# wolearyc/ramannoodle

Measured on AMD Instinct MI355X. Metric: structures/sec (GNN polarizability eval), higher is better.
Workload: dtype f32

## Files before the change

### ramannoodle_amd/csrc/kernels_edge_ps.hip

```cpp
#include <algorithm>
#include <vector>

#include "fused_common.hpp"

namespace rn {

struct EdgePsArgs {
  const float *edge_in;
  float *edge_out;
  const float *node;
  const float *np3;
  float *agg_out;
  int *fail;
  int S;
  Graph g;
  Dims d;
  PassW<float> w;
};

#ifndef RN_PS_TIMING
#define RN_PS_TIMING 0
#endif
#ifndef RN_PS_PROBE
#define RN_PS_PROBE 0
#endif
#ifndef RN_PS_SLEEP
#define RN_PS_SLEEP 1
#endif
#ifndef RN_PS_PRIO
#define RN_PS_PRIO 3
#endif
#ifndef RN_PS_CPRIO
#define RN_PS_CPRIO 2
#endif
#ifndef RN_PS_LG8
#define RN_PS_LG8 1
#endif
#ifndef RN_PS_TICKET
#define RN_PS_TICKET 1
#endif
#ifndef RN_PS_LPRIO
#define RN_PS_LPRIO 1
#endif
#if RN_PS_TIMING
#define PS_T0() long long _t = (long long)__builtin_readcyclecounter(); ++tn
#define PS_TICK(i)                                                                       \
  do {                                                                                   \
    const long long _n = (long long)__builtin_readcyclecounter();                        \
    tl[(i) & 15] += (unsigned)(_n - _t);                                                 \
    _t = (long long)__builtin_readcyclecounter();                                        \
  } while (0)
#define PS_TFLUSH(first, last, shift)                                                    \
  do {                                                                                   \
    if (timed)                                                                           \
      for (int _i = (first); _i <= (last); ++_i) {                                       \
        tacc[2 * (_i + (shift))] += (long long)tl[_i & 15];                              \
        tacc[2 * (_i + (shift)) + 1] += (long long)tn;                                   \
      }                                                                                  \
  } while (0)
#else
#define PS_T0() do {} while (0)
#define PS_TICK(i) do {} while (0)
#define PS_TFLUSH(first, last, shift) do {} while (0)
#endif

namespace {
constexpr int PS_THREADS = 768;
constexpr int PS_PROD = 4;
constexpr int PS_ND = 16;
#ifndef RN_PS_NRT
#define RN_PS_NRT 8
#endif
constexpr int PS_NRT = RN_PS_NRT;
constexpr int PS_NRT_GRAM = 7;
constexpr int PS_GW = 3;
constexpr int PS_GSTRIDE = PS_GW * 16 * 16;
constexpr int PS_MAXNEW = 2;
constexpr int PS_TILE = 16 * FP;
constexpr int PS_BUF = (2 + PS_MAXNEW) * PS_TILE;

constexpr int PS_CSET = 4;
constexpr unsigned PS_FAILBIT = 0x80000000u;

enum { C_SPLIT = 0, C_NORM = 16, C_READY = 32, C_FREE0 = 48, C_FREE1 = 64, C_RD0 = 80, C_RD1 = 96, C_TICKET = 112 };

struct PsLds {
  size_t ring, qnp, bufP, bufC, atile, lnp, ints, sync, gram, total;
};
__host__ __device__ inline PsLds ps_lds(int maxR, int maxD, bool gram) {
  auto up = [](size_t b) { return (b + 15) & ~size_t(15); };
  const size_t maxR16 = ((size_t)maxR + 15) & ~size_t(15), rounds = ((size_t)maxD + PS_ND - 1) / PS_ND;
  PsLds L;
  size_t off = 0;
  const size_t ring_rows = (size_t)(gram ? PS_NRT_GRAM : PS_NRT) * 16;
  L.ring = off; off += ring_rows * LDQ * 4;
  L.qnp = off; off += ring_rows * 4 * 4;
  L.bufP = off; off += (size_t)2 * PS_ND * LDQ * 4;
  L.bufC = off; off += (size_t)2 * PS_ND * LDQ * 4;
  L.atile = off; off += ((size_t)2 * PS_BUF + PS_TILE) * 4;
  L.lnp = off; off += (size_t)(gram ? 6 : 16) * FP * 4;
  L.ints = off; off += up((maxR16 + 7 * (size_t)maxD + 2 * rounds + 8) * 4);
  L.sync = off; off += 128;
  L.gram = off; off += gram ? (size_t)2 * PS_PROD * PS_GSTRIDE * 4 : 0;
  L.total = off;
  return L;
}

struct PsStep {
  int has_dest;
  int u, r, g;
  int ntiles, tile0;
  int tu0, tt0, tu1, tt1;
  int slot0, slot1;
  int ubs;
};
struct PsSched {
  int nrounds, nrt, nunits;
  int P, pu, pt;
  int u, r, g;
  int h0, hc;
  int ring, ps, ubs;
};
__host__ __device__ inline int ps_wrap(int x, int ring) { return x >= ring ? x - ring : x; }
__host__ __device__ inline void ps_sched_init(PsSched &s, int nrounds, int nrt, int nunits, int hi0, int ring) {
  s.nrounds = nrounds;
  s.nrt = nrt;
  s.nunits = nunits;
  s.P = s.pu = s.pt = s.u = s.r = s.g = 0;
  s.h0 = s.hc = hi0;
  s.ring = ring;
  s.ps = s.ubs = 0;
}
__host__ __device__ inline void ps_sched_take(PsSched &s, PsStep &st, int n) {
  st.ntiles = n;
  st.tile0 = s.P;
  st.tu0 = st.tu1 = s.pu;
  st.tt0 = st.tt1 = s.pt;
  st.slot0 = st.slot1 = s.ps;
  if (n >= 1) {
    ++s.P;
    s.ps = ps_wrap(s.ps + 1, s.ring);
    if (++s.pt == s.nrt) { s.pt = 0; ++s.pu; }
  }
  if (n >= 2) {
    st.tu1 = s.pu;
    st.tt1 = s.pt;
    st.slot1 = s.ps;
    ++s.P;
    s.ps = ps_wrap(s.ps + 1, s.ring);
    if (++s.pt == s.nrt) { s.pt = 0; ++s.pu; }
  }
}
template <typename HiFn>
__host__ __device__ inline bool ps_sched_next(PsSched &s, HiFn hi, PsStep &st) {
  if (s.u >= s.nunits) return false;
  if (s.g == 0 && s.P < s.h0 + 1) {
    const int miss = s.h0 + 1 - s.P;
    st.has_dest = 0;
    st.u = st.r = st.g = 0;
    st.ubs = 0;
    ps_sched_take(s, st, miss < PS_MAXNEW ? miss : PS_MAXNEW);
    return true;
  }
  const int need_now = s.u * s.nrt + s.hc + 1;
  int u2 = s.u, r2 = s.r + 1;
  if (r2 == s.nrounds) { r2 = 0; ++u2; }
  const int h2 = r2 == 0 ? s.h0 : hi(r2);
  const int need_next = u2 < s.nunits ? u2 * s.nrt + h2 + 1 : need_now;
  int n = need_next - s.P;
  n = n < 0 ? 0 : (n > PS_MAXNEW ? PS_MAXNEW : n);
  if (n < need_now - s.P) n = need_now - s.P;
  st.has_dest = 1;
  st.u = s.u;
  st.r = s.r;
  st.g = s.g;
  st.ubs = s.ubs;
  ps_sched_take(s, st, n);
  if (u2 != s.u) {
    int b = s.ubs + s.nrt % s.ring;
    s.ubs = ps_wrap(b, s.ring);
  }
  s.u = u2;
  s.r = r2;
  s.hc = h2;
  ++s.g;
  return true;
}

__device__ __forceinline__ unsigned ps_wait_ge(unsigned word, unsigned target, unsigned ready_word, int *fail, int code) {
  for (unsigned spins = 0;; ++spins) {
    unsigned v;
    asm volatile("ds_read_b32 %0, %1\n\ts_waitcnt lgkmcnt(0)" : "=v"(v) : "v"(word) : "memory");
    v = (unsigned)__builtin_amdgcn_readfirstlane((int)v);
    if (v >= target) return v;
    bool give_up = spins > (1u << 21);
    if ((spins & 1023u) == 1023u && !give_up) {
      unsigned rv;
      asm volatile("ds_read_b32 %0, %1\n\ts_waitcnt lgkmcnt(0)" : "=v"(rv) : "v"(ready_word) : "memory");
      give_up = ((unsigned)__builtin_amdgcn_readfirstlane((int)rv) & PS_FAILBIT) != 0;
    }
    if (give_up) {
      *fail = code;
      asm volatile("ds_or_b32 %0, %1\n\ts_waitcnt vmcnt(0) lgkmcnt(0)" ::"v"(ready_word), "v"(PS_FAILBIT) : "memory");
      return v | PS_FAILBIT;
    }
#if RN_PS_SLEEP
    __builtin_amdgcn_s_sleep(RN_PS_SLEEP);
#endif
  }
}
__device__ __forceinline__ void ps_arrive(unsigned word, int lane) {
  asm volatile("s_waitcnt lgkmcnt(0)" ::: "memory");
  if (lane == 0) asm volatile("ds_add_u32 %0, %1" ::"v"(word), "v"(1u) : "memory");
}
__device__ __forceinline__ unsigned ps_arrive_ticket(unsigned word, int lane) {
  asm volatile("s_waitcnt lgkmcnt(0)" ::: "memory");
  unsigned old = 0;
  if (lane == 0) asm volatile("ds_add_rtn_u32 %0, %1, %2\n\ts_waitcnt lgkmcnt(0)" : "=&v"(old) : "v"(word), "v"(1u) : "memory");
  return (unsigned)__builtin_amdgcn_readfirstlane((int)old);
}
typedef __bf16 bf16x8 __attribute__((ext_vector_type(8)));
typedef __bf16 bf16x2 __attribute__((ext_vector_type(2)));
__device__ __forceinline__ void split_bf16x8(const f32x4 &x0, const f32x4 &x1, bf16x8 &hi, bf16x8 &lo) {
#pragma unroll
  for (int j = 0; j < 4; ++j) {
    const f32x2 v = j < 2 ? f32x2{x0[2 * j], x0[2 * j + 1]} : f32x2{x1[2 * j - 4], x1[2 * j - 3]};
    const bf16x2 h = __builtin_convertvector(v, bf16x2);
    const bf16x2 l = __builtin_convertvector(v - __builtin_convertvector(h, f32x2), bf16x2);
    hi[2 * j] = h[0];
    hi[2 * j + 1] = h[1];
    lo[2 * j] = l[0];
    lo[2 * j + 1] = l[1];
  }
}
__device__ __forceinline__ void ps_publish(unsigned word, unsigned value, int lane) {
  asm volatile("s_waitcnt lgkmcnt(0)" ::: "memory");
  if (lane == 0) asm volatile("ds_max_u32 %0, %1" ::"v"(word), "v"(value) : "memory");
}
}

template <bool PAD, bool PRE, bool GRAM, bool F16 = true>
__global__ __launch_bounds__(PS_THREADS) void edge_block_ps_kernel(EdgePsArgs a) {
  static_assert(F16 || (!PRE && !GRAM), "the exact-f32 instantiation keeps float32 rows and the in-loop cross term");
  extern __shared__ __attribute__((aligned(16))) unsigned char smem_raw[];
  constexpr int NRT = GRAM ? PS_NRT_GRAM : PS_NRT, RING = NRT * 16;
  constexpr bool LG8 = RN_PS_LG8 && !GRAM;
  constexpr unsigned CPR = LG8 ? 2u : (unsigned)PS_CSET;
  auto wrap_row = [](unsigned x) -> unsigned {
    if constexpr ((RING & (RING - 1)) == 0) return x & (unsigned)(RING - 1);
    else return min(x, x - (unsigned)RING);
  };
  const Graph &g = a.g;
  const PsLds L = ps_lds(g.pt_max_out_rows, g.pt_max_in_rows, GRAM);
  auto wsc = [&](int i) { return F16 ? a.w.mfma_scale_c[i] : 1.0f; };
  float *ring = reinterpret_cast<float *>(smem_raw + L.ring);
  float *qnp = reinterpret_cast<float *>(smem_raw + L.qnp);
  float *bufP = reinterpret_cast<float *>(smem_raw + L.bufP);
  float *bufC = reinterpret_cast<float *>(smem_raw + L.bufC);
  float *atile = reinterpret_cast<float *>(smem_raw + L.atile);
  float *na_tile = atile + 2 * PS_BUF;
  float *lnp = reinterpret_cast<float *>(smem_raw + L.lnp);
  float *s_c2b = lnp, *s_g3q = lnp + 2 * FP, *s_igp = lnp + 4 * FP;
  float *s_g3p = lnp + 6 * FP, *s_c21g = lnp + 8 * FP, *s_c21b = lnp + 10 * FP, *s_c22g = lnp + 12 * FP, *s_c22b = lnp + 13 * FP,
        *s_c3g = lnp + 14 * FP, *s_c3b = lnp + 15 * FP;
  int *ints = reinterpret_cast<int *>(smem_raw + L.ints);
  unsigned *sync = reinterpret_cast<unsigned *>(smem_raw + L.sync);
  const unsigned sync_a = lds_addr(sync);
  const unsigned atile_a = lds_addr(atile), lnp_a = lds_addr(lnp), qnp_a = lds_addr(qnp), ints_a = lds_addr(ints);
  const unsigned bufP_a = lds_addr(bufP), ring_a = lds_addr(ring);
  float *gram_f = reinterpret_cast<float *>(smem_raw + L.gram);
  const int maxD = g.pt_max_in_rows, maxR16 = (g.pt_max_out_rows + 15) & ~15;
  int *qb = ints;
  int *d_edge = qb + maxR16, *d_a = d_edge + maxD, *d_b = d_a + maxD, *d_rb = d_b + maxD, *d_cnt = d_rb + maxD,
      *d_skip = d_cnt + maxD, *d_re = d_skip + maxD;
  int *hi_t = d_re + maxD;
  int *lo_t = hi_t + (maxD + PS_ND - 1) / PS_ND;
  int *misc = lo_t + (maxD + PS_ND - 1) / PS_ND;
  const int hi_off = maxR16 + 7 * maxD;
  const int lo_off = hi_off + (maxD + PS_ND - 1) / PS_ND;

  const int tid = threadIdx.x, lane = tid & 63;
  const int wave = __builtin_amdgcn_readfirstlane(tid >> 6);
  const int l15 = lane & 15, quad = lane >> 4;

  int logical = blockIdx.x;
  if ((gridDim.x & 7) == 0) logical = (blockIdx.x & 7) * (gridDim.x >> 3) + (blockIdx.x >> 3);
  const int tile = logical % g.pt_num;
  const int sg = logical / g.pt_num, nsg = gridDim.x / g.pt_num;
  const int j0 = g.pt_begin[tile], j1 = g.pt_begin[tile + 1];
  const int eo0 = g.out_ptr[j0], R = g.out_ptr[j1] - eo0;
  const int di0 = g.in_ptr[j0], D = g.in_ptr[j1] - di0;
  const int nrounds = (D + PS_ND - 1) / PS_ND;
  const int back = g.pt_back;

  for (int c = tid; c < 2 * FP; c += PS_THREADS) {
    s_c2b[c] = a.w.c2_bias_c[c] * wsc(4);
    const float gam = a.w.c3_norm_1s.g[c];
    s_g3q[c] = gam * wsc(3);
    s_igp[c] = ((c % FP) < a.d.Fe) ? wsc(1) / gam * (1.0f / (float)a.d.Fe) : 0.0f;
    if constexpr (!GRAM) {
      s_g3p[c] = gam * wsc(1);
      s_c21g[c] = a.w.c2_norm_1.g[c];
      s_c21b[c] = a.w.c2_norm_1.b[c];
      if (c < FP) {
        s_c22g[c] = a.w.c2_norm_2.g[c];
        s_c22b[c] = a.w.c2_norm_2.b[c];
        s_c3g[c] = a.w.c3_norm_2.g[c];
        s_c3b[c] = a.w.c3_norm_2.b[c];
      }
    }
  }
  for (int r = tid; r < maxR16; r += PS_THREADS) qb[r] = g.edge_b[eo0 + min(r, max(R - 1, 0))];
  for (int i = tid; i < D; i += PS_THREADS) {
    const int dst = g.in_edge[di0 + i];
    const int ad = g.edge_a[dst], bd = g.edge_b[dst];
    const int rb = g.out_ptr[bd] - eo0, re = g.out_ptr[bd + 1] - eo0;
    const int rev = g.rev_edge[dst];
    d_edge[i] = dst;
    d_a[i] = ad;
    d_b[i] = bd;
    d_rb[i] = rb;
    d_cnt[i] = (re - rb) - (rev >= 0 ? 1 : 0);
    d_skip[i] = rev >= 0 ? rev - eo0 : re;
    d_re[i] = re;
  }
  if (tid < 32) sync[tid] = 0u;
  __syncthreads();
  if (tid < nrounds) {
    int top = 0, first = 1 << 30;
    const int last = min((tid + 1) * PS_ND, D);
    for (int i = 0; i < last; ++i) {
      top = max(top, d_re[i]);
      if (i >= tid * PS_ND && d_re[i] > d_rb[i]) first = min(first, d_rb[i]);
    }
    hi_t[tid] = (top + 15) / 16 - 1;
    lo_t[tid] = first == (1 << 30) ? (top + 15) / 16 : first / 16;
  }
  __syncthreads();
  if (tid == 0) misc[0] = max(hi_t[nrounds > 0 ? nrounds - 1 : 0] + 1, 1);
  __syncthreads();
  if (D == 0 || sg >= a.S) return;
  const int nrt = __builtin_amdgcn_readfirstlane(misc[0]);
  const int nunits = (a.S - sg + nsg - 1) / nsg;

  if (wave < PS_PROD) {
    __builtin_amdgcn_s_setprio(RN_PS_PRIO);
    const int colbase = wave * 32;
    auto uni = [](float v) { return __int_as_float(__builtin_amdgcn_readfirstlane(__float_as_int(v))); };
    const float s4 = uni(wsc(0));
    const float s5 = uni(wsc(2)), inv5 = uni(wsc(3));
    const float sc2 = uni(wsc(4));
    WaveB<F16> bW4, bW5, bWc;
    bW4.load(a.w.c3_WeT_c, 4 * FP, colbase, l15, quad, s4);
    bW5.load(a.w.c3_WeT_c + 2 * FP, 4 * FP, colbase, l15, quad, s5);
    bWc.load(a.w.c2_WT_c, 2 * FP, colbase, l15, quad, sc2);
    const float qscale = uni(inv5 * inv5 / (float)(2 * a.d.Fe));

    auto request = [&](const PsStep &st, int buf, int ln) {
      const int row = 4 * wave + (ln >> 4);
      const int piece = ((ln & 15) ^ row) & 15;
      float *dst = atile + buf * PS_BUF + wave * 256;
      const unsigned ia = ints_a + (unsigned)(maxR16 + min(st.r * PS_ND + row, D - 1)) * 4u;
      int de, da, db;
      lds_read1x3(ia, ia + (unsigned)maxD * 4u, ia + 2u * (unsigned)maxD * 4u, de, da, db);
      const int s = sg + st.u * nsg;
      const float *eb = a.edge_in + (int64_t)s * g.E * FP, *nb = a.node + (int64_t)s * g.N * FP;
      const float *eb0 = a.edge_in + (int64_t)(sg + min(st.tu0, nunits - 1) * nsg) * g.E * FP;
      const float *eb1 = a.edge_in + (int64_t)(sg + min(st.tu1, nunits - 1) * nsg) * g.E * FP;
      const unsigned r0 = (unsigned)(eo0 + min(st.tt0 * 16 + row, R - 1)), r1 = (unsigned)(eo0 + min(st.tt1 * 16 + row, R - 1));
      dma16(eb + ((unsigned)de * FP + 4 * piece), dst);
      dma16(nb + ((unsigned)db * FP + 4 * piece), dst + PS_TILE);
      dma16(nb + ((unsigned)da * FP + 4 * piece), na_tile + wave * 256);
      dma16(eb0 + (r0 * FP + 4 * piece), dst + 2 * PS_TILE);
      dma16(eb1 + (r1 * FP + 4 * piece), dst + 3 * PS_TILE);
    };
    auto split_landed = [&](int buf, int ln) {
      const int row = 4 * wave + (ln >> 4), phys = ln & 15;
      const unsigned tb = atile_a + (unsigned)(buf * PS_BUF) * 4u;
      const unsigned sa = tb + (unsigned)(wave * 256 + ln * 4) * 4u;
      f32x4 u, v, w;
      if constexpr (!PRE && F16) {
        lds_read3(sa, sa + 2 * PS_TILE * 4, sa + 3 * PS_TILE * 4, u, v, w);
        write_pair(tb, row, phys, u);
        write_pair(tb + 2 * PS_TILE * 4, row, phys, v);
        write_pair(tb + 3 * PS_TILE * 4, row, phys, w);
      }
      lds_read2(sa + PS_TILE * 4, atile_a + (unsigned)(2 * PS_BUF + wave * 256 + ln * 4) * 4u, u, v);
// ... 96 lines not shown
        asm volatile("global_load_dwordx4 %0, %1, off" : "=v"(qS[1]) : "v"(q_src + 16) : "memory");
      }
      if (cur.has_dest) {
        f32x4 accC[2];
        if constexpr (F16) {
          f16x8 ah[2], al[2];
          load_pair_a2(tb_a + PS_TILE * 4, l15, quad, ah, al, lnp_a + (unsigned)mycol * 4u, lnp_a + (unsigned)(mycol + 16) * 4u,
                       accC[0], accC[1]);
          if (!(RN_PS_PROBE & 2)) bWc.product_split(ah, al, accC);
        } else {
          float af[KS];
          load_f32_a2(tb_a + PS_TILE * 4, l15, quad, af, lnp_a + (unsigned)mycol * 4u, lnp_a + (unsigned)(mycol + 16) * 4u, accC[0], accC[1]);
          if (!(RN_PS_PROBE & 2)) bWc.product(af, accC);
        }
#pragma unroll
        for (int t = 0; t < 2; ++t)
          *reinterpret_cast<f32x4 *>(bufC + (slot0 + l15) * LDQ + mycol + 16 * t) = accC[t];
      }
      PS_TICK(6);
      const int ntl = (RN_PS_PROBE & 128) ? 0 : cur.ntiles;
      auto q_tile_finish = [&](f32x4 (&accQ)[2], const f32x4 (&g3v)[2], int ringrow) {
#pragma unroll
        for (int t = 0; t < 2; ++t) accQ[t] = qS[t] * s5 + accQ[t];
        float ss = 0.f;
#pragma unroll
        for (int t = 0; t < 2; ++t)
#pragma unroll
          for (int e = 0; e < 4; ++e) ss = fmaf(accQ[t][e], accQ[t][e], ss);
        ss = sum_xor32(sum_xor16(ss));
#pragma unroll
        for (int t = 0; t < 2; ++t) *reinterpret_cast<f32x4 *>(ring + ringrow * LDQ + mycol + 16 * t) = accQ[t] * g3v[t];
        if (quad == 0) qnp[ringrow * 4 + wave] = ss * qscale;
      };
      {
        f32x4 accQ[2] = {{0.f, 0.f, 0.f, 0.f}, {0.f, 0.f, 0.f, 0.f}}, g3v[2] = {{0.f, 0.f, 0.f, 0.f}, {0.f, 0.f, 0.f, 0.f}};
        if (ntl > 0) {
          if constexpr (F16) {
            f16x8 ah[2], al[2];
            load_pair_a2(tb_a + (unsigned)(2 * PS_TILE) * 4u, l15, quad, ah, al, lnp_a + (unsigned)(2 * FP + mycol) * 4u,
                         lnp_a + (unsigned)(2 * FP + mycol + 16) * 4u, g3v[0], g3v[1]);
            if (!(RN_PS_PROBE & 2)) bW5.product_split(ah, al, accQ);
          } else {
            float af[KS];
            load_f32_a2(tb_a + (unsigned)(2 * PS_TILE) * 4u, l15, quad, af, lnp_a + (unsigned)(2 * FP + mycol) * 4u,
                        lnp_a + (unsigned)(2 * FP + mycol + 16) * 4u, g3v[0], g3v[1]);
            if (!(RN_PS_PROBE & 2)) bW5.product(af, accQ);
          }
        }
        asm volatile("s_waitcnt vmcnt(0)" : "+v"(qS[0]), "+v"(qS[1]), "+v"(accQ[0]), "+v"(accQ[1])::"memory");
        PS_TICK(7);
        if (cur.has_dest && cur.g > back) {
          const int gdone = cur.g - back - 1;
          ps_wait_ge(sync_a + ((gdone & 1) ? C_RD1 : C_RD0), CPR * (unsigned)((gdone >> 1) + 1), sync_a + C_READY, a.fail, 3);
        }
        PS_TICK(9);
        if (ntl > 0) q_tile_finish(accQ, g3v, ringrow0);
      }
      if (ntl > 1) {
        const float *np3_q = a.np3 + (int64_t)(sg + min(cur.tu1, nunits - 1) * nsg) * g.N * (6 * FP);
        const unsigned oq = (unsigned)lds_read1(ints_a + (unsigned)min(cur.tt1 * 16 + l15, R - 1) * 4u) * (6 * FP) + mycol;
#pragma unroll
        for (int t = 0; t < 2; ++t) qS[t] = *reinterpret_cast<const f32x4 *>(np3_q + oq + 16 * t);
        f32x4 accQ[2] = {{0.f, 0.f, 0.f, 0.f}, {0.f, 0.f, 0.f, 0.f}}, g3v[2];
        if constexpr (F16) {
          f16x8 ah[2], al[2];
          load_pair_a2(tb_a + (unsigned)(3 * PS_TILE) * 4u, l15, quad, ah, al, lnp_a + (unsigned)(2 * FP + mycol) * 4u,
                       lnp_a + (unsigned)(2 * FP + mycol + 16) * 4u, g3v[0], g3v[1]);
          if (!(RN_PS_PROBE & 2)) bW5.product_split(ah, al, accQ);
        } else {
          float af[KS];
          load_f32_a2(tb_a + (unsigned)(3 * PS_TILE) * 4u, l15, quad, af, lnp_a + (unsigned)(2 * FP + mycol) * 4u,
                      lnp_a + (unsigned)(2 * FP + mycol + 16) * 4u, g3v[0], g3v[1]);
          if (!(RN_PS_PROBE & 2)) bW5.product(af, accQ);
        }
        q_tile_finish(accQ, g3v, cur.slot1 * 16 + l15);
      }
      if constexpr (GRAM) {
        if (cur.has_dest) {
          const unsigned prow_a = bufP_a + (unsigned)((slot0 + l15) * LDQ + mycol) * 4u;
          const unsigned ig_a = lnp_a + (unsigned)(4 * FP + mycol) * 4u;
          const int lo = __builtin_amdgcn_readfirstlane(lds_read1(ints_a + (unsigned)(lo_off + cur.r) * 4u));
          const int hiw = __builtin_amdgcn_readfirstlane(lds_read1(ints_a + (unsigned)(hi_off + cur.r) * 4u));
          unsigned qa[PS_GW];
#pragma unroll
          for (int k = 0; k < PS_GW; ++k) {
            int sl = cur.ubs + min(lo + k, max(hiw, lo));
            sl = sl >= NRT ? sl - NRT : sl;
            sl = sl >= NRT ? sl - NRT : sl;
            qa[k] = ring_a + (unsigned)((sl * 16 + l15) * LDQ + mycol) * 4u;
          }
          static_assert(PS_GW == 3, "the Gram phase is written for three window tiles");
          f32x4 p0, p1, i0, i1, q0[PS_GW], q1[PS_GW];
          asm volatile(
              "ds_read_b128 %0, %10\n\tds_read_b128 %1, %10 offset:64\n\tds_read_b128 %2, %11\n\tds_read_b128 %3, %11 offset:64\n\t"
              "ds_read_b128 %4, %12\n\tds_read_b128 %5, %12 offset:64\n\tds_read_b128 %6, %13\n\tds_read_b128 %7, %13 offset:64\n\t"
              "ds_read_b128 %8, %14\n\tds_read_b128 %9, %14 offset:64\n\ts_waitcnt lgkmcnt(0)"
              : "=&v"(p0), "=&v"(p1), "=&v"(i0), "=&v"(i1), "=&v"(q0[0]), "=&v"(q1[0]), "=&v"(q0[1]), "=&v"(q1[1]), "=&v"(q0[2]), "=&v"(q1[2])
              : "v"(prow_a), "v"(ig_a), "v"(qa[0]), "v"(qa[1]), "v"(qa[2])
              : "memory");
          bf16x8 ph, pl, qh[PS_GW], ql[PS_GW];
          split_bf16x8(p0 * i0, p1 * i1, ph, pl);
#pragma unroll
          for (int k = 0; k < PS_GW; ++k) split_bf16x8(q0[k], q1[k], qh[k], ql[k]);
          f32x4 gacc[PS_GW];
#pragma unroll
          for (int k = 0; k < PS_GW; ++k) gacc[k] = __builtin_amdgcn_mfma_f32_16x16x32_bf16(pl, qh[k], f32x4{0.f, 0.f, 0.f, 0.f}, 0, 0, 0);
#pragma unroll
          for (int k = 0; k < PS_GW; ++k) gacc[k] = __builtin_amdgcn_mfma_f32_16x16x32_bf16(ph, ql[k], gacc[k], 0, 0, 0);
#pragma unroll
          for (int k = 0; k < PS_GW; ++k) gacc[k] = __builtin_amdgcn_mfma_f32_16x16x32_bf16(ph, qh[k], gacc[k], 0, 0, 0);
          const int gout = ((cur.g & 1) * PS_PROD + wave) * PS_GSTRIDE + l15 * 16 + 4 * quad;
#pragma unroll
          for (int k = 0; k < PS_GW; ++k) *reinterpret_cast<f32x4 *>(gram_f + gout + k * 256) = gacc[k];
        }
      }
      PS_TICK(7);
      if (ps_arrive_ticket(sync_a + C_NORM, ln) == 4u * k + 3u) {
        if (ln < 16 * cur.ntiles) {
          const int rrow = ((ln >> 4) ? cur.slot1 : cur.slot0) * 16 + l15;
          f32x4 v, v2;
          lds_read2(qnp_a + (unsigned)rrow * 16u, qnp_a + (unsigned)rrow * 16u, v, v2);
          ring[rrow * LDQ + 2 * FP] = (v[0] + v[1]) + (v[2] + v[3]);
        }
        if (cur.has_dest) ps_publish(sync_a + C_READY, (unsigned)cur.g + 1u, ln);
      }
      PS_TICK(8);
      cur = nxt;
      have = have_next;
    }
    dma_wait();
    PS_TFLUSH(0, 9, 0);
    return;
  }

  const int cw = wave - PS_PROD;
  if constexpr (LG8) {
    const int l7 = lane & 7, grp = lane >> 3;
    const float inv2n = 1.0f / (float)(2 * a.d.Fe), invn = 1.0f / (float)a.d.Fe;
    const float spscale = wsc(1) * wsc(1) * inv2n;
    const float eps_c2 = 1e-5f * wsc(4) * wsc(4);
    int nval[2];
#pragma unroll
    for (int j = 0; j < 2; ++j) nval[j] = min(max(a.d.Fe - (4 * l7 + 32 * j), 0), 4);
    f32x2 bf2[2][2], bc2[2][2];
#pragma unroll
    for (int j = 0; j < 2; ++j) {
      const Vec4<float> bf = load4<float>(a.w.c3_norm_1s.b + 4 * l7 + 32 * j), bc = load4<float>(a.w.c3_norm_1s.b + FP + 4 * l7 + 32 * j);
      bf2[j][0] = f32x2{bf.v[0], bf.v[1]};
      bf2[j][1] = f32x2{bf.v[2], bf.v[3]};
      bc2[j][0] = f32x2{bc.v[0], bc.v[1]};
      bc2[j][1] = f32x2{bc.v[2], bc.v[3]};
      asm volatile("s_waitcnt vmcnt(0)" : "+v"(bf2[j][0]), "+v"(bf2[j][1]), "+v"(bc2[j][0]), "+v"(bc2[j][1]));
    }
    const float *ringc = ring + 4 * l7;
    const int sdelta = 2 * FP - 4 * l7;
    const unsigned total_rounds = (unsigned)nunits * (unsigned)nrounds;
    auto ln64 = [&](const Vec4<float> (&x)[2], const float *gt, const float *bt, Vec4<float> (&y)[2]) {
      float sum = 0.f;
#pragma unroll
      for (int j = 0; j < 2; ++j) sum += (x[j].v[0] + x[j].v[1]) + (x[j].v[2] + x[j].v[3]);
      const float mean = lg_sum<8>(sum) * invn;
      float dv[2][4], qq = 0.f;
#pragma unroll
      for (int j = 0; j < 2; ++j)
#pragma unroll
        for (int k = 0; k < 4; ++k) {
          dv[j][k] = x[j].v[k] - mean;
          if (PAD && k >= nval[j]) dv[j][k] = 0.f;
          qq = fmaf(dv[j][k], dv[j][k], qq);
        }
      const float rstd = fast_rsq(lg_sum<8>(qq) * invn + 1e-5f);
#pragma unroll
      for (int j = 0; j < 2; ++j) {
        const Vec4<float> gv = load4<float>(gt + 4 * l7 + 32 * j), bv = load4<float>(bt + 4 * l7 + 32 * j);
#pragma unroll
        for (int k = 0; k < 4; ++k) y[j].v[k] = dv[j][k] * rstd * gv.v[k] + bv.v[k];
      }
    };
    bool poisoned = false;
#if RN_PS_TIMING
    long long *tacc = reinterpret_cast<long long *>(a.fail + 16);
    const bool timed = blockIdx.x == 0 && (cw & 3) == 0 && lane == 0;
    unsigned tl[16] = {0, 0, 0, 0, 0, 0, 0, 0, 0, 0, 0, 0, 0, 0, 0, 0}, tn = 0;
#endif
    for (;;) {
      PS_T0();
      const unsigned tk = ps_arrive_ticket(sync_a + C_TICKET, lane);
      const unsigned gr = tk >> 1;
      if (gr >= total_rounds) break;
      const int slot = 8 * (int)(tk & 1u) + grp;
      const int u = (int)(gr / (unsigned)nrounds), r = (int)(gr - (unsigned)u * (unsigned)nrounds);
      const int ub = (int)(((unsigned)u * (unsigned)(nrt % NRT)) % (unsigned)NRT) * 16;
      poisoned |= (ps_wait_ge(sync_a + C_READY, gr + 1u, sync_a + C_READY, a.fail, 4) & PS_FAILBIT) != 0;
      PS_TICK(10);
      const int64_t erow0 = (int64_t)(sg + u * nsg) * g.E;
      const bool active = r * PS_ND + slot < D;
      const int i = min(r * PS_ND + slot, D - 1);
      const int64_t drow = erow0 + d_edge[i];
      f32x2 pf2[2][2], pc2[2][2], pdf2[2][2], pdc2[2][2];
      float spe;
      {
        const float *prow = bufP + ((int)(gr & 1u) * PS_ND + slot) * LDQ;
        float sp = 0.f;
#pragma unroll
        for (int j = 0; j < 2; ++j) {
          const int cj = 4 * l7 + 32 * j;
          const Vec4<float> xf = load4<float>(prow + cj), xc = load4<float>(prow + FP + cj);
          const Vec4<float> gf = load4<float>(s_g3p + cj), gc = load4<float>(s_g3p + FP + cj);
          const Vec4<float> jf = load4<float>(s_igp + cj), jc = load4<float>(s_igp + FP + cj);
#pragma unroll
          for (int k = 0; k < 4; ++k) sp += xf.v[k] * xf.v[k] + xc.v[k] * xc.v[k];
#pragma unroll
          for (int hh = 0; hh < 2; ++hh) {
            pdf2[j][hh] = f32x2{xf.v[2 * hh] * jf.v[2 * hh], xf.v[2 * hh + 1] * jf.v[2 * hh + 1]};
            pdc2[j][hh] = f32x2{xc.v[2 * hh] * jc.v[2 * hh], xc.v[2 * hh + 1] * jc.v[2 * hh + 1]};
            pf2[j][hh] = f32x2{xf.v[2 * hh] * gf.v[2 * hh], xf.v[2 * hh + 1] * gf.v[2 * hh + 1]};
            pc2[j][hh] = f32x2{xc.v[2 * hh] * gc.v[2 * hh], xc.v[2 * hh + 1] * gc.v[2 * hh + 1]};
          }
        }
        spe = lg_sum<8>(sp) * spscale + 1e-5f;
      }
      Vec4<float> c2v[2];
      {
        const float *crow = bufC + ((int)(gr & 1u) * PS_ND + slot) * LDQ;
        Vec4<float> xf[2], xc[2];
        float q = 0.f;
#pragma unroll
        for (int j = 0; j < 2; ++j) {
          xf[j] = load4<float>(crow + 4 * l7 + 32 * j);
          xc[j] = load4<float>(crow + FP + 4 * l7 + 32 * j);
#pragma unroll
          for (int k = 0; k < 4; ++k) q += xf[j].v[k] * xf[j].v[k] + xc[j].v[k] * xc[j].v[k];
        }
        const float rstd2 = fast_rsq(lg_sum<8>(q) * inv2n + eps_c2);
        Vec4<float> g2[2];
#pragma unroll
        for (int j = 0; j < 2; ++j) {
          const int cj = 4 * l7 + 32 * j;
          const Vec4<float> gf = load4<float>(s_c21g + cj), bf = load4<float>(s_c21b + cj);
          const Vec4<float> gc = load4<float>(s_c21g + FP + cj), bc = load4<float>(s_c21b + FP + cj);
#pragma unroll
          for (int k = 0; k < 4; ++k)
            g2[j].v[k] = (RN_PS_PROBE & 4) ? xf[j].v[k] + xc[j].v[k]
                                           : gate(xf[j].v[k] * rstd2 * gf.v[k] + bf.v[k], xc[j].v[k] * rstd2 * gc.v[k] + bc.v[k]);
        }
        if (RN_PS_PROBE & 4) {
          c2v[0] = g2[0];
          c2v[1] = g2[1];
        } else {
          ln64(g2, s_c22g, s_c22b, c2v);
        }
      }
      const int rb = d_rb[i], cnt = active ? d_cnt[i] : 0, rskip = d_skip[i];
      const int rbase = (int)wrap_row(wrap_row((unsigned)(ub + rb)));
      ps_arrive(sync_a + ((gr & 1u) ? C_FREE1 : C_FREE0), lane);
      PS_TICK(11);
      float acc[8] = {0.f, 0.f, 0.f, 0.f, 0.f, 0.f, 0.f, 0.f};
      {
        auto triplet = [&](const float *qr, float (&sumk)[8]) {
          f32x2 qf2[2][2], qc2[2][2];
#pragma unroll
          for (int j = 0; j < 2; ++j) {
            const float4 qfv = *reinterpret_cast<const float4 *>(qr + 32 * j), qcv = *reinterpret_cast<const float4 *>(qr + FP + 32 * j);
            qf2[j][0] = f32x2{qfv.x, qfv.y};
            qf2[j][1] = f32x2{qfv.z, qfv.w};
            qc2[j][0] = f32x2{qcv.x, qcv.y};
            qc2[j][1] = f32x2{qcv.z, qcv.w};
          }
          const float qs = qr[sdelta];
          f32x2 d2 = pdf2[0][0] * qf2[0][0], d3 = pdc2[0][0] * qc2[0][0];
          d2 = __builtin_elementwise_fma(pdf2[0][1], qf2[0][1], d2);
          d3 = __builtin_elementwise_fma(pdc2[0][1], qc2[0][1], d3);
          d2 = __builtin_elementwise_fma(pdf2[1][0], qf2[1][0], d2);
          d3 = __builtin_elementwise_fma(pdc2[1][0], qc2[1][0], d3);
          d2 = __builtin_elementwise_fma(pdf2[1][1], qf2[1][1], d2);
          d3 = __builtin_elementwise_fma(pdc2[1][1], qc2[1][1], d3);
          d2 += d3;
          const float dot = lg_sum<8>(d2.x + d2.y);
          float ve = dot + (spe + qs);
          ve = ve > 1e-5f ? ve : 1e-5f;
          const float rstd = fast_rsq(ve);
          const f32x2 rstd2 = {rstd, rstd}, one2 = {1.0f, 1.0f};
#pragma unroll
          for (int j = 0; j < 2; ++j)
#pragma unroll
            for (int hh = 0; hh < 2; ++hh) {
              const f32x2 xf2 = __builtin_elementwise_fma(pf2[j][hh] + qf2[j][hh], rstd2, bf2[j][hh]);
              const f32x2 xc2 = __builtin_elementwise_fma(pc2[j][hh] + qc2[j][hh], rstd2, bc2[j][hh]);
              const f32x2 e1 = {fast_exp2(xf2.x), fast_exp2(xf2.y)}, e2 = {fast_exp2(xc2.x), fast_exp2(xc2.y)};
              const f32x2 t2 = e2 + one2;
              const f32x2 den = __builtin_elementwise_fma(e1, t2, t2);
              const f32x2 rd = {fast_rcp(den.x), fast_rcp(den.y)};
              f32x2 sk = {sumk[4 * j + 2 * hh], sumk[4 * j + 2 * hh + 1]};
              sk = __builtin_elementwise_fma(e2 - one2, rd, sk);
              sumk[4 * j + 2 * hh] = sk.x;
              sumk[4 * j + 2 * hh + 1] = sk.y;
            }
        };
#if RN_PS_CPRIO
        __builtin_amdgcn_s_setprio(0);
#endif
        float acc2[8] = {0.f, 0.f, 0.f, 0.f, 0.f, 0.f, 0.f, 0.f};
        const int tskip = rskip - rb;
        auto row_of = [&](int t) { return ringc + __umul24(wrap_row((unsigned)(rbase + t + (t >= tskip ? 1 : 0))), (unsigned)LDQ); };
        int t = (RN_PS_PROBE & 1) ? cnt : 0;
        const int tmid = RN_PS_LPRIO ? ((cnt >> 1) & ~1) : 0;
        for (; t + 1 < tmid; t += 2) {
          triplet(row_of(t), acc);
          triplet(row_of(t + 1), acc2);
        }
#if RN_PS_LPRIO
        __builtin_amdgcn_s_setprio(RN_PS_LPRIO);
#endif
        for (; t + 1 < cnt; t += 2) {
          triplet(row_of(t), acc);
          triplet(row_of(t + 1), acc2);
        }
        if (t < cnt) triplet(row_of(t), acc);
#pragma unroll
        for (int k = 0; k < 8; ++k) acc[k] += acc2[k];
      }
      PS_TICK(12);
#if RN_PS_CPRIO
      __builtin_amdgcn_s_setprio(RN_PS_CPRIO);
#endif
      f32x4 old4[2];
#pragma unroll
      for (int j = 0; j < 2; ++j) {
        const int cj = 4 * l7 + 32 * j;
        if constexpr (PRE) {
          const char *pp = reinterpret_cast<const char *>(a.edge_in + drow * FP + (cj >> 3) * 8) + (cj & 7) * 2;
          const f16x4 hh = *reinterpret_cast<const f16x4 *>(pp), ll = *reinterpret_cast<const f16x4 *>(pp + 16);
#pragma unroll
          for (int k = 0; k < 4; ++k) old4[j][k] = (float)hh[k] + (float)ll[k];
        } else {
          old4[j] = *reinterpret_cast<const f32x4 *>(a.edge_in + drow * FP + cj);
        }
      }
      poisoned |= (ps_wait_ge(sync_a + ((gr & 1u) ? C_RD1 : C_RD0), CPR * (gr >> 1), sync_a + C_READY, a.fail, 6) & PS_FAILBIT) != 0;
      ps_arrive(sync_a + ((gr & 1u) ? C_RD1 : C_RD0), lane);
      if (active) {
        Vec4<float> a4[2], c3[2];
#pragma unroll
        for (int j = 0; j < 2; ++j) {
          a4[j] = Vec4<float>{{acc[4 * j], acc[4 * j + 1], acc[4 * j + 2], acc[4 * j + 3]}};
          if (a.agg_out) store4(a.agg_out + drow * FP + 4 * l7 + 32 * j, a4[j]);
        }
        if (RN_PS_PROBE & 4) {
          c3[0] = a4[0];
          c3[1] = a4[1];
        } else {
          ln64(a4, s_c3g, s_c3b, c3);
        }
#pragma unroll
        for (int j = 0; j < 2; ++j) {
          const int cj = 4 * l7 + 32 * j;
          f32x4 y;
#pragma unroll
          for (int k = 0; k < 4; ++k) {
            y[k] = (RN_PS_PROBE & 4) ? old4[j][k] + c2v[j].v[k] + c3[j].v[k] : fast_tanh(old4[j][k] + c2v[j].v[k] + c3[j].v[k]);
            if (poisoned) y[k] = __int_as_float(0x7fc00000);
          }
          if constexpr (PRE) {
            char *pp = reinterpret_cast<char *>(a.edge_out + drow * FP + (cj >> 3) * 8) + (cj & 7) * 2;
            f16x4 hh, ll;
#pragma unroll
            for (int k = 0; k < 4; ++k) {
              hh[k] = (_Float16)y[k];
              ll[k] = (_Float16)(y[k] - (float)hh[k]);
            }
            *reinterpret_cast<f16x4 *>(pp) = hh;
            *reinterpret_cast<f16x4 *>(pp + 16) = ll;
          } else {
            *reinterpret_cast<f32x4 *>(a.edge_out + drow * FP + cj) = y;
          }
        }
      }
      PS_TICK(13);
    }
    PS_TFLUSH(10, 13, (cw >> 2) ? 6 : 0);
    return;
  }
  const int cset = cw >> 2;
  const int c0 = 4 * l15;
  const int nvalid = min(max(a.d.Fe - c0, 0), 4);
  const float inv2n = 1.0f / (float)(2 * a.d.Fe), invn = 1.0f / (float)a.d.Fe;
  const float spscale = wsc(1) * wsc(1) * inv2n;
  const float eps_c2 = 1e-5f * wsc(4) * wsc(4);
  f32x2 bf2[2], bc2[2];
  {
    const Vec4<float> bf = load4<float>(a.w.c3_norm_1s.b + c0), bc = load4<float>(a.w.c3_norm_1s.b + FP + c0);
    bf2[0] = f32x2{bf.v[0], bf.v[1]};
    bf2[1] = f32x2{bf.v[2], bf.v[3]};
    bc2[0] = f32x2{bc.v[0], bc.v[1]};
    bc2[1] = f32x2{bc.v[2], bc.v[3]};
    asm volatile("s_waitcnt vmcnt(0)" : "+v"(bf2[0]), "+v"(bf2[1]), "+v"(bc2[0]), "+v"(bc2[1]));
  }
  LnParams<float> k_c3 = {load4<float>(a.w.c3_norm_2.g + c0), load4<float>(a.w.c3_norm_2.b + c0)};
  LnParams<float> k_c21f = {load4<float>(a.w.c2_norm_1.g + c0), load4<float>(a.w.c2_norm_1.b + c0)};
  LnParams<float> k_c21c = {load4<float>(a.w.c2_norm_1.g + FP + c0), load4<float>(a.w.c2_norm_1.b + FP + c0)};
  LnParams<float> k_c22 = {load4<float>(a.w.c2_norm_2.g + c0), load4<float>(a.w.c2_norm_2.b + c0)};
  Vec4<float> g3f = load4<float>(a.w.c3_norm_1s.g + c0), g3c = load4<float>(a.w.c3_norm_1s.g + FP + c0);
  {
    auto pin = [](Vec4<float> &x) { asm volatile("s_waitcnt vmcnt(0)" : "+v"(x.v[0]), "+v"(x.v[1]), "+v"(x.v[2]), "+v"(x.v[3])); };
    pin(k_c3.g); pin(k_c3.b); pin(k_c21f.g); pin(k_c21f.b); pin(k_c21c.g); pin(k_c21c.b); pin(k_c22.g); pin(k_c22.b);
    pin(g3f); pin(g3c);
  }
#pragma unroll
  for (int k = 0; k < 4; ++k) {
    g3f.v[k] *= wsc(1);
    g3c.v[k] *= wsc(1);
  }
  Vec4<float> igf = load4<float>(s_igp + c0), igc = load4<float>(s_igp + FP + c0);
  const float *ringc = ring + c0;
  const int sdelta = 2 * FP - c0;
  const unsigned total_rounds = (unsigned)nunits * (unsigned)nrounds;
  auto locate = [&](unsigned gr, int &u, int &r, int &ub) {
    u = (int)(gr / (unsigned)nrounds);
    r = (int)(gr - (unsigned)u * (unsigned)nrounds);
    ub = (int)(((unsigned)u * (unsigned)(nrt % NRT)) % (unsigned)NRT) * 16;
  };
  int u = 0, r = 0, ub = 0;
  bool poisoned = false;
#if RN_PS_TIMING
  long long *tacc = reinterpret_cast<long long *>(a.fail + 16);
  const bool timed = blockIdx.x == 0 && (cw & 3) == 0 && lane == 0;
  unsigned tl[16] = {0, 0, 0, 0, 0, 0, 0, 0, 0, 0, 0, 0, 0, 0, 0, 0}, tn = 0;
#endif
  for (unsigned turn = 0;; ++turn) {
    PS_T0();
    unsigned gr;
    int slot;
    if (RN_PS_TICKET) {
      const unsigned q = ps_arrive_ticket(sync_a + C_TICKET, lane);
      gr = q >> 2;
      slot = 4 * (int)(q & 3u) + quad;
    } else {
      gr = 2u * turn + (unsigned)cset;
      slot = 4 * (cw & 3) + quad;
    }
    if (gr >= total_rounds) break;
    locate(gr, u, r, ub);
    poisoned |= (ps_wait_ge(sync_a + C_READY, gr + 1u, sync_a + C_READY, a.fail, 4) & PS_FAILBIT) != 0;
    PS_TICK(10);
    const int64_t erow0 = (int64_t)(sg + u * nsg) * g.E;
    const bool active = r * PS_ND + slot < D;
    const int i = min(r * PS_ND + slot, D - 1);
    const int64_t drow = erow0 + d_edge[i];
    f32x4 old4;
    if constexpr (PRE) {
      const char *pp = reinterpret_cast<const char *>(a.edge_in + drow * FP + (c0 >> 3) * 8) + (c0 & 7) * 2;
      const f16x4 hh = *reinterpret_cast<const f16x4 *>(pp), ll = *reinterpret_cast<const f16x4 *>(pp + 16);
#pragma unroll
      for (int k = 0; k < 4; ++k) old4[k] = (float)hh[k] + (float)ll[k];
    } else {
      old4 = *reinterpret_cast<const f32x4 *>(a.edge_in + drow * FP + c0);
    }
    f32x2 pf2[2], pc2[2], pdf2[2], pdc2[2];
    float spe;
    {
      const float *prow = bufP + ((int)(gr & 1u) * PS_ND + slot) * LDQ;
      const Vec4<float> xf = load4<float>(prow + c0), xc = load4<float>(prow + FP + c0);
      float sp = 0.f;
#pragma unroll
      for (int k = 0; k < 4; ++k) sp += xf.v[k] * xf.v[k] + xc.v[k] * xc.v[k];
      sp = lg_sum<LG>(sp);
#pragma unroll
      for (int hh = 0; hh < 2; ++hh) {
        if constexpr (!GRAM) {
          pdf2[hh] = f32x2{xf.v[2 * hh] * igf.v[2 * hh], xf.v[2 * hh + 1] * igf.v[2 * hh + 1]};
          pdc2[hh] = f32x2{xc.v[2 * hh] * igc.v[2 * hh], xc.v[2 * hh + 1] * igc.v[2 * hh + 1]};
        }
        pf2[hh] = f32x2{xf.v[2 * hh] * g3f.v[2 * hh], xf.v[2 * hh + 1] * g3f.v[2 * hh + 1]};
        pc2[hh] = f32x2{xc.v[2 * hh] * g3c.v[2 * hh], xc.v[2 * hh + 1] * g3c.v[2 * hh + 1]};
      }
      spe = sp * spscale + 1e-5f;
    }
    Vec4<float> c2v;
    {
      const float *crow = bufC + ((int)(gr & 1u) * PS_ND + slot) * LDQ;
      const Vec4<float> xf = load4<float>(crow + c0), xc = load4<float>(crow + FP + c0);
      float q = 0.f;
#pragma unroll
      for (int k = 0; k < 4; ++k) q += xf.v[k] * xf.v[k] + xc.v[k] * xc.v[k];
      const float rstd2 = fast_rsq(lg_sum<LG>(q) * inv2n + eps_c2);
      Vec4<float> g2;
#pragma unroll
      for (int k = 0; k < 4; ++k) {
        g2.v[k] = (RN_PS_PROBE & 4) ? xf.v[k] + xc.v[k]
                                    : gate(xf.v[k] * rstd2 * k_c21f.g.v[k] + k_c21f.b.v[k], xc.v[k] * rstd2 * k_c21c.g.v[k] + k_c21c.b.v[k]);
      }
      c2v = (RN_PS_PROBE & 4) ? g2 : ln_row<LG, PAD, float>(g2, k_c22, invn, nvalid);
    }
    const int rb = d_rb[i], cnt = active ? d_cnt[i] : 0, rskip = d_skip[i];
    const int rbase = (int)wrap_row(wrap_row((unsigned)(ub + rb)));
    float rs0 = 0.f, rs1 = 0.f;
    if constexpr (GRAM) {
      const int nrow = d_re[i] - rb;
      const int lo_r = __builtin_amdgcn_readfirstlane(lo_t[r]);
      const float *gtab = reinterpret_cast<const float *>(smem_raw + L.gram) + (int)(gr & 1u) * (PS_PROD * PS_GSTRIDE) + slot;
#pragma unroll
      for (int pass = 0; pass < 2; ++pass) {
        const int er = min(l15 + 16 * pass, max(nrow - 1, 0));
        const int urow = rb + er;
        const int tl = min(max((urow >> 4) - lo_r, 0), PS_GW - 1);
        const float *gp = gtab + (tl * 16 + (urow & 15)) * 16;
        const float qs = ring[wrap_row((unsigned)(rbase + er)) * LDQ + 2 * FP];
#ifdef RN_PS_GRAM_DEBUG
        float gsum = 0.f;
// ... 199 lines not shown
```

Measured before the change: 63450.

## Precompute per-wave ring row address tables in LDS for the triplet loop

In the LG8 consumer path, each wave now writes a small LDS table of ring row byte addresses in chunks of 24 neighbours and walks it with paired 64-bit LDS loads. Layer-norm and gate parameters are read through a single laundered LDS base address with fixed offsets instead of separate pointers. Topology values are reloaded per chunk, and scheduling barriers are placed between phases. The aim is to lower VGPR pressure and the per-iteration address arithmetic (wrap and skip logic) in the hot inner loop. The cost is extra LDS traffic, extra LDS space and wave barriers for each chunk.

```diff
diff --git a/ramannoodle_amd/csrc/kernels_edge_ps.hip b/ramannoodle_amd/csrc/kernels_edge_ps.hip
--- a/ramannoodle_amd/csrc/kernels_edge_ps.hip
+++ b/ramannoodle_amd/csrc/kernels_edge_ps.hip
@@ -38,6 +38,9 @@
 #endif
 #ifndef RN_PS_TICKET
 #define RN_PS_TICKET 1
+#endif
+#ifndef RN_PS_ROWTAB
+#define RN_PS_ROWTAB 1
 #endif
 #ifndef RN_PS_LPRIO
 #define RN_PS_LPRIO 1
@@ -64,6 +67,12 @@
 #define PS_TFLUSH(first, last, shift) do {} while (0)
 #endif
 
+#if RN_PS_ROWTAB
+#define PS_SCHED_FENCE() __builtin_amdgcn_sched_barrier(0)
+#else
+#define PS_SCHED_FENCE() do {} while (0)
+#endif
+
 namespace {
 constexpr int PS_THREADS = 768;
 constexpr int PS_PROD = 4;
@@ -79,13 +88,14 @@
 constexpr int PS_TILE = 16 * FP;
 constexpr int PS_BUF = (2 + PS_MAXNEW) * PS_TILE;
 
+constexpr int PS_TC = 24;
 constexpr int PS_CSET = 4;
 constexpr unsigned PS_FAILBIT = 0x80000000u;
 
 enum { C_SPLIT = 0, C_NORM = 16, C_READY = 32, C_FREE0 = 48, C_FREE1 = 64, C_RD0 = 80, C_RD1 = 96, C_TICKET = 112 };
 
 struct PsLds {
-  size_t ring, qnp, bufP, bufC, atile, lnp, ints, sync, gram, total;
+  size_t ring, qnp, bufP, bufC, atile, lnp, ints, sync, gram, rowtab, total;
 };
 __host__ __device__ inline PsLds ps_lds(int maxR, int maxD, bool gram) {
   auto up = [](size_t b) { return (b + 15) & ~size_t(15); };
@@ -102,6 +112,7 @@
   L.ints = off; off += up((maxR16 + 7 * (size_t)maxD + 2 * rounds + 8) * 4);
   L.sync = off; off += 128;
   L.gram = off; off += gram ? (size_t)2 * PS_PROD * PS_GSTRIDE * 4 : 0;
+  L.rowtab = off; off += (!gram && RN_PS_LG8 && RN_PS_ROWTAB) ? (size_t)8 * 8 * PS_TC * 4 + 16 : 0;
   L.total = off;
   return L;
 }
@@ -233,6 +244,12 @@
     lo[2 * j + 1] = l[1];
   }
 }
+typedef const __attribute__((address_space(3))) float *lds_cfp;
+__device__ __forceinline__ f32x4 ld4(const float *p) { return *reinterpret_cast<const f32x4 *>(p); }
+__device__ __forceinline__ f32x4 ld4(lds_cfp p) { return *reinterpret_cast<const __attribute__((address_space(3))) f32x4 *>(p); }
+__device__ __forceinline__ lds_cfp lds_f(unsigned a) { return reinterpret_cast<lds_cfp>(a); }
+typedef unsigned u32x2 __attribute__((ext_vector_type(2)));
+__device__ __forceinline__ u32x2 ld2(unsigned a) { return *reinterpret_cast<const __attribute__((address_space(3))) u32x2 *>(a); }
 __device__ __forceinline__ void ps_publish(unsigned word, unsigned value, int lane) {
   asm volatile("s_waitcnt lgkmcnt(0)" ::: "memory");
   if (lane == 0) asm volatile("ds_max_u32 %0, %1" ::"v"(word), "v"(value) : "memory");
@@ -635,10 +652,21 @@
       bc2[j][1] = f32x2{bc.v[2], bc.v[3]};
       asm volatile("s_waitcnt vmcnt(0)" : "+v"(bf2[j][0]), "+v"(bf2[j][1]), "+v"(bc2[j][0]), "+v"(bc2[j][1]));
     }
+#if !RN_PS_ROWTAB
     const float *ringc = ring + 4 * l7;
     const int sdelta = 2 * FP - 4 * l7;
+#endif
     const unsigned total_rounds = (unsigned)nunits * (unsigned)nrounds;
-    auto ln64 = [&](const Vec4<float> (&x)[2], const float *gt, const float *bt, Vec4<float> (&y)[2]) {
+    [[maybe_unused]] unsigned lt_a = 0;
+    auto tl4 = [&](int off) -> Vec4<float> {
+#if RN_PS_ROWTAB
+      const f32x4 v = ld4(lds_f(lt_a) + off);
+      return Vec4<float>{{v[0], v[1], v[2], v[3]}};
+#else
+      return load4<float>(lnp + 4 * l7 + off);
+#endif
+    };
+    auto ln64 = [&](const Vec4<float> (&x)[2], int gt, int bt, Vec4<float> (&y)[2]) {
       float sum = 0.f;
 #pragma unroll
       for (int j = 0; j < 2; ++j) sum += (x[j].v[0] + x[j].v[1]) + (x[j].v[2] + x[j].v[3]);
@@ -655,7 +683,7 @@
       const float rstd = fast_rsq(lg_sum<8>(qq) * invn + 1e-5f);
 #pragma unroll
       for (int j = 0; j < 2; ++j) {
-        const Vec4<float> gv = load4<float>(gt + 4 * l7 + 32 * j), bv = load4<float>(bt + 4 * l7 + 32 * j);
+        const Vec4<float> gv = tl4(gt + 32 * j), bv = tl4(bt + 32 * j);
 #pragma unroll
         for (int k = 0; k < 4; ++k) y[j].v[k] = dv[j][k] * rstd * gv.v[k] + bv.v[k];
       }
@@ -672,6 +700,7 @@
       const unsigned gr = tk >> 1;
       if (gr >= total_rounds) break;
       const int slot = 8 * (int)(tk & 1u) + grp;
+      lt_a = (unsigned)launder((int)(lnp_a + 16u * (unsigned)l7));
       const int u = (int)(gr / (unsigned)nrounds), r = (int)(gr - (unsigned)u * (unsigned)nrounds);
       const int ub = (int)(((unsigned)u * (unsigned)(nrt % NRT)) % (unsigned)NRT) * 16;
       poisoned |= (ps_wait_ge(sync_a + C_READY, gr + 1u, sync_a + C_READY, a.fail, 4) & PS_FAILBIT) != 0;
@@ -689,8 +718,8 @@
         for (int j = 0; j < 2; ++j) {
           const int cj = 4 * l7 + 32 * j;
           const Vec4<float> xf = load4<float>(prow + cj), xc = load4<float>(prow + FP + cj);
-          const Vec4<float> gf = load4<float>(s_g3p + cj), gc = load4<float>(s_g3p + FP + cj);
-          const Vec4<float> jf = load4<float>(s_igp + cj), jc = load4<float>(s_igp + FP + cj);
+          const Vec4<float> gf = tl4(6 * FP + 32 * j), gc = tl4(7 * FP + 32 * j);
+          const Vec4<float> jf = tl4(4 * FP + 32 * j), jc = tl4(5 * FP + 32 * j);
 #pragma unroll
           for (int k = 0; k < 4; ++k) sp += xf.v[k] * xf.v[k] + xc.v[k] * xc.v[k];
 #pragma unroll
@@ -703,6 +732,7 @@
         }
         spe = lg_sum<8>(sp) * spscale + 1e-5f;
       }
+      PS_SCHED_FENCE();
       Vec4<float> c2v[2];
       {
         const float *crow = bufC + ((int)(gr & 1u) * PS_ND + slot) * LDQ;
@@ -719,9 +749,8 @@
         Vec4<float> g2[2];
 #pragma unroll
         for (int j = 0; j < 2; ++j) {
-          const int cj = 4 * l7 + 32 * j;
-          const Vec4<float> gf = load4<float>(s_c21g + cj), bf = load4<float>(s_c21b + cj);
-          const Vec4<float> gc = load4<float>(s_c21g + FP + cj), bc = load4<float>(s_c21b + FP + cj);
+          const Vec4<float> gf = tl4(8 * FP + 32 * j), bf = tl4(10 * FP + 32 * j);
+          const Vec4<float> gc = tl4(9 * FP + 32 * j), bc = tl4(11 * FP + 32 * j);
 #pragma unroll
           for (int k = 0; k < 4; ++k)
             g2[j].v[k] = (RN_PS_PROBE & 4) ? xf[j].v[k] + xc[j].v[k]
@@ -731,26 +760,29 @@
           c2v[0] = g2[0];
           c2v[1] = g2[1];
         } else {
-          ln64(g2, s_c22g, s_c22b, c2v);
-        }
-      }
+          ln64(g2, 12 * FP, 13 * FP, c2v);
+        }
+      }
+      PS_SCHED_FENCE();
+#if !RN_PS_ROWTAB
       const int rb = d_rb[i], cnt = active ? d_cnt[i] : 0, rskip = d_skip[i];
       const int rbase = (int)wrap_row(wrap_row((unsigned)(ub + rb)));
+#endif
       ps_arrive(sync_a + ((gr & 1u) ? C_FREE1 : C_FREE0), lane);
       PS_TICK(11);
       float acc[8] = {0.f, 0.f, 0.f, 0.f, 0.f, 0.f, 0.f, 0.f};
       {
-        auto triplet = [&](const float *qr, float (&sumk)[8]) {
+        auto triplet = [&](auto qr, auto qsp, float (&sumk)[8]) {
           f32x2 qf2[2][2], qc2[2][2];
 #pragma unroll
           for (int j = 0; j < 2; ++j) {
-            const float4 qfv = *reinterpret_cast<const float4 *>(qr + 32 * j), qcv = *reinterpret_cast<const float4 *>(qr + FP + 32 * j);
-            qf2[j][0] = f32x2{qfv.x, qfv.y};
-            qf2[j][1] = f32x2{qfv.z, qfv.w};
-            qc2[j][0] = f32x2{qcv.x, qcv.y};
-            qc2[j][1] = f32x2{qcv.z, qcv.w};
+            const f32x4 qfv = ld4(qr + 32 * j), qcv = ld4(qr + FP + 32 * j);
+            qf2[j][0] = f32x2{qfv[0], qfv[1]};
+            qf2[j][1] = f32x2{qfv[2], qfv[3]};
+            qc2[j][0] = f32x2{qcv[0], qcv[1]};
+            qc2[j][1] = f32x2{qcv[2], qcv[3]};
           }
-          const float qs = qr[sdelta];
+          const float qs = *qsp;
           f32x2 d2 = pdf2[0][0] * qf2[0][0], d3 = pdc2[0][0] * qc2[0][0];
           d2 = __builtin_elementwise_fma(pdf2[0][1], qf2[0][1], d2);
           d3 = __builtin_elementwise_fma(pdc2[0][1], qc2[0][1], d3);
@@ -784,22 +816,69 @@
         __builtin_amdgcn_s_setprio(0);
 #endif
         float acc2[8] = {0.f, 0.f, 0.f, 0.f, 0.f, 0.f, 0.f, 0.f};
+#if !RN_PS_ROWTAB
         const int tskip = rskip - rb;
+        const int tmid = RN_PS_LPRIO ? ((cnt >> 1) & ~1) : 0;
+#endif
+#if RN_PS_ROWTAB
+        const int lz = launder(lane), l7 = lz & 7;
+        unsigned tp = lds_addr(smem_raw + L.rowtab) + (unsigned)((cw * 8 + (lz >> 3)) * PS_TC) * 4u;
+        const unsigned topo_a = ints_a + (unsigned)(maxR16 + 3 * maxD + i) * 4u;
+        for (int t0 = (RN_PS_PROBE & 1) ? (1 << 30) : 0;; t0 += PS_TC) {
+          int rb, cnt, rskip;
+          lds_read1x3(topo_a, topo_a + (unsigned)maxD * 4u, topo_a + 2u * (unsigned)maxD * 4u, rb, cnt, rskip);
+          if (!active) cnt = 0;
+          if (t0 >= cnt) break;
+          if (t0 > 0) tp -= 4u * PS_TC;
+          const int rbase = (int)wrap_row(wrap_row((unsigned)(ub + rb)));
+          const int tskip = rskip - rb;
+          __builtin_amdgcn_wave_barrier();
+#pragma unroll
+          for (int k = 0; k < PS_TC / 8; ++k) {
+            const int te = t0 + l7 + 8 * k;
+            const unsigned ra = ring_a + __umul24(wrap_row((unsigned)(rbase + te + (te >= tskip ? 1 : 0))), (unsigned)(LDQ * 4));
+            *reinterpret_cast<__attribute__((address_space(3))) unsigned *>(tp + 4u * (unsigned)(l7 + 8 * k)) = ra;
+          }
+          __builtin_amdgcn_wave_barrier();
+          const int tmid = RN_PS_LPRIO ? ((cnt >> 1) & ~1) : 0;
+          const int n = min(cnt - t0, PS_TC), nmid = min(max(tmid - t0, 0), n);
+          const unsigned end_mid = tp + 4u * (unsigned)nmid, end_pairs = tp + 4u * (unsigned)(n & ~1);
+          const bool odd = (n & 1) != 0;
+          u32x2 nx = ld2(tp);
+          auto pair = [&]() {
+            const u32x2 cu = nx;
+            triplet(lds_f(cu.x) + 4 * l7, lds_f(cu.x) + 2 * FP, acc);
+            triplet(lds_f(cu.y) + 4 * l7, lds_f(cu.y) + 2 * FP, acc2);
+            tp += 8;
+            nx = ld2(tp);
+          };
+#if RN_PS_LPRIO && RN_PS_CPRIO
+          __builtin_amdgcn_s_setprio(0);
+#endif
+          while (tp < end_mid) pair();
+#if RN_PS_LPRIO
+          __builtin_amdgcn_s_setprio(RN_PS_LPRIO);
+#endif
+          while (tp < end_pairs) pair();
+          if (odd) triplet(lds_f(nx.x) + 4 * l7, lds_f(nx.x) + 2 * FP, acc);
+          if (cnt <= t0 + PS_TC) break;
+        }
+#else
         auto row_of = [&](int t) { return ringc + __umul24(wrap_row((unsigned)(rbase + t + (t >= tskip ? 1 : 0))), (unsigned)LDQ); };
         int t = (RN_PS_PROBE & 1) ? cnt : 0;
-        const int tmid = RN_PS_LPRIO ? ((cnt >> 1) & ~1) : 0;
         for (; t + 1 < tmid; t += 2) {
-          triplet(row_of(t), acc);
-          triplet(row_of(t + 1), acc2);
+          triplet(row_of(t), row_of(t) + sdelta, acc);
+          triplet(row_of(t + 1), row_of(t + 1) + sdelta, acc2);
         }
 #if RN_PS_LPRIO
         __builtin_amdgcn_s_setprio(RN_PS_LPRIO);
 #endif
         for (; t + 1 < cnt; t += 2) {
-          triplet(row_of(t), acc);
-          triplet(row_of(t + 1), acc2);
-        }
-        if (t < cnt) triplet(row_of(t), acc);
+          triplet(row_of(t), row_of(t) + sdelta, acc);
+          triplet(row_of(t + 1), row_of(t + 1) + sdelta, acc2);
+        }
+        if (t < cnt) triplet(row_of(t), row_of(t) + sdelta, acc);
+#endif
 #pragma unroll
         for (int k = 0; k < 8; ++k) acc[k] += acc2[k];
       }
@@ -807,10 +886,11 @@
 #if RN_PS_CPRIO
       __builtin_amdgcn_s_setprio(RN_PS_CPRIO);
 #endif
+      const int l7e = RN_PS_ROWTAB ? (launder(lane) & 7) : l7;
       f32x4 old4[2];
 #pragma unroll
       for (int j = 0; j < 2; ++j) {
-        const int cj = 4 * l7 + 32 * j;
+        const int cj = 4 * l7e + 32 * j;
         if constexpr (PRE) {
           const char *pp = reinterpret_cast<const char *>(a.edge_in + drow * FP + (cj >> 3) * 8) + (cj & 7) * 2;
           const f16x4 hh = *reinterpret_cast<const f16x4 *>(pp), ll = *reinterpret_cast<const f16x4 *>(pp + 16);
@@ -827,17 +907,17 @@
 #pragma unroll
         for (int j = 0; j < 2; ++j) {
           a4[j] = Vec4<float>{{acc[4 * j], acc[4 * j + 1], acc[4 * j + 2], acc[4 * j + 3]}};
-          if (a.agg_out) store4(a.agg_out + drow * FP + 4 * l7 + 32 * j, a4[j]);
+          if (a.agg_out) store4(a.agg_out + drow * FP + 4 * l7e + 32 * j, a4[j]);
         }
         if (RN_PS_PROBE & 4) {
           c3[0] = a4[0];
           c3[1] = a4[1];
         } else {
-          ln64(a4, s_c3g, s_c3b, c3);
+          ln64(a4, 14 * FP, 15 * FP, c3);
         }
 #pragma unroll
         for (int j = 0; j < 2; ++j) {
-          const int cj = 4 * l7 + 32 * j;
+          const int cj = 4 * l7e + 32 * j;
           f32x4 y;
 #pragma unroll
           for (int k = 0; k < 4; ++k) {
```

Result: no change. 63760, median of 6 (+0.5%).
